# ORNL/DDStore

Hardware: AMD Instinct MI355X
Metric: samples/sec (global-shuffle sample fetch) (higher is better)
Workload: dtype bf16; 1 GPU; model=store-globalshuffle-fetch, global_batch=262144, rows_per_rank=2097152, row_bytes=512, store_dtype=f32, parallelism=dp1, mode=fetch

## Files before the change

ddstore_amd/csrc/ddstore_kernels.hip:

```cpp

#include "ddstore_kernels.h"

#include <hip/hip_fp16.h>
#include <hip/hip_bf16.h>
#include <hip/hip_fp8.h>
#include <type_traits>
#include <cstdlib>
#include <string>

namespace ddstore {

namespace {

constexpr int kBlock = 256;
constexpr int64_t kMaxBlocks = 32768;

inline int n_blocks(int64_t work_items) {
    int64_t b = (work_items + kBlock - 1) / kBlock;
    if (b < 1) b = 1;
    if (b > kMaxBlocks) b = kMaxBlocks;
    return (int)b;
}

template <typename T, int N>
struct alignas(sizeof(T) * N) VecT {
    T v[N];
};

__device__ __forceinline__ int owner_of(const int64_t* prefix, int nparts, int64_t row) {
    int lo = 0, hi = nparts - 1;
    while (lo < hi) {
        int mid = (lo + hi + 1) >> 1;
        if (prefix[mid] <= row) lo = mid; else hi = mid - 1;
    }
    return lo;
}

template <typename P, int NPFX = 1>
struct LdsDir {
    int64_t prefix[NPFX][DDS_MAX_PARTS + 1];
    P base[DDS_MAX_PARTS];

    __device__ __forceinline__ void load(const void* const* peer_base, int nparts,
                                         const int64_t* gprefix0,
                                         const int64_t* gprefix1 = nullptr) {
        for (int i = threadIdx.x; i <= nparts; i += kBlock) {
            prefix[0][i] = gprefix0[i];
            if constexpr (NPFX == 2) prefix[1][i] = gprefix1[i];
        }
        for (int i = threadIdx.x; i < nparts; i += kBlock)
            base[i] = reinterpret_cast<P>(peer_base[i]);
        __syncthreads();
    }
};

template <typename P, int NPFX>
__device__ __forceinline__ int owner_of(const LdsDir<P, NPFX>& d, int nparts, int64_t row) {
    return owner_of(d.prefix[0], nparts, row);
}

template <typename P, int NPFX>
__device__ __forceinline__ bool out_of_range(const LdsDir<P, NPFX>& d, int nparts,
                                             int64_t g) {
    return g < 0 || g >= d.prefix[0][nparts];
}

template <typename T>
constexpr bool is_fp8_v =
    std::is_same_v<T, __hip_fp8_e4m3> || std::is_same_v<T, __hip_fp8_e5m2>;

__device__ __forceinline__ float f64_to_f32(double v) {
#pragma clang fp contract(off)
    return static_cast<float>(v);
}

template <typename Tout, typename Tin>
__device__ __forceinline__ Tout cvt(Tin v) {
    if constexpr (std::is_same_v<Tout, Tin>) {
        return v;
    } else if constexpr (std::is_same_v<Tin, double> &&
                         (std::is_same_v<Tout, __half> ||
                          std::is_same_v<Tout, __hip_bfloat16>)) {
        return cvt<Tout, float>(f64_to_f32(v));
    } else if constexpr (std::is_same_v<Tout, uint8_t> &&
                         std::is_floating_point_v<Tin>) {
        return static_cast<uint8_t>(static_cast<int32_t>(v));
    } else if constexpr (std::is_same_v<Tin, __half>) {
        return cvt<Tout, float>(__half2float(v));
    } else if constexpr (std::is_same_v<Tin, __hip_bfloat16>) {
        return cvt<Tout, float>(__bfloat162float(v));
    } else if constexpr (is_fp8_v<Tin>) {
        return cvt<Tout, float>(static_cast<float>(v));
    } else if constexpr (std::is_same_v<Tout, __half>) {
        return __float2half(static_cast<float>(v));
    } else if constexpr (std::is_same_v<Tout, __hip_bfloat16>) {
        return __float2bfloat16(static_cast<float>(v));
    } else if constexpr (is_fp8_v<Tout>) {
        const float f = static_cast<float>(v);
        Tout r(f);
        if constexpr (std::is_same_v<Tout, __hip_fp8_e4m3>) {
            if (fabsf(f) > 464.0f) r.__x = 0x7F;
        } else {
            if (fabsf(f) >= 61440.0f) r.__x = f < 0.0f ? 0xFC : 0x7C;
        }
        return r;
    } else {
        return static_cast<Tout>(v);
    }
}

struct XfIdentity {
    template <typename Tout, typename Tin>
    __device__ __forceinline__ Tout apply(Tin v) const { return v; }
};
struct XfCast {
    template <typename Tout, typename Tin>
    __device__ __forceinline__ Tout apply(Tin v) const { return cvt<Tout>(v); }
};
struct XfAffine {
    float scale, shift;
    uint32_t opaque_zero = 0;
    template <typename Tout, typename Tin>
    __device__ __forceinline__ Tout apply(Tin v) const {
        float y = fmaf(cvt<float>(v), scale, shift);
        if constexpr (std::is_same_v<Tout, __half>)
            y = __uint_as_float(__float_as_uint(y) | opaque_zero);
        return cvt<Tout>(y);
    }
};

template <typename Tin, typename Tout, int VEC, typename Xf>
__global__ void __launch_bounds__(kBlock)
k_gather_oneshot(const void* const* peer_base, const int64_t* gprefix, int nparts,
                 const int64_t* idx, int64_t nidx, int64_t row_elems, Xf xf,
                 Tout* __restrict__ out, unsigned long long* oob) {
    using Vin = VecT<Tin, VEC>;
    using Vout = VecT<Tout, VEC>;
    __shared__ LdsDir<const Tin*> dir;
    dir.load(peer_base, nparts, gprefix);

    const int64_t cpr = row_elems / VEC;
    const int64_t total = nidx * cpr;
    for (int64_t t = (int64_t)blockIdx.x * kBlock + threadIdx.x; t < total;
         t += (int64_t)gridDim.x * kBlock) {
        const int64_t r = t / cpr;
        const int64_t c = t - r * cpr;
        const int64_t g = idx[r];
        if (out_of_range(dir, nparts, g)) {
            if (c == 0) atomicAdd(oob, 1ull);
            continue;
        }
        const int p = owner_of(dir, nparts, g);
        const Vin vin = *reinterpret_cast<const Vin*>(
            dir.base[p] + (g - dir.prefix[0][p]) * row_elems + c * VEC);
        Vout vout;
#pragma unroll
        for (int k = 0; k < VEC; ++k) vout.v[k] = xf.template apply<Tout>(vin.v[k]);
        *reinterpret_cast<Vout*>(out + t * VEC) = vout;
    }
}

typedef uint32_t dds_u32x4 __attribute__((ext_vector_type(4)));
typedef uint32_t dds_u32x2 __attribute__((ext_vector_type(2)));
#define DDS_GLOBAL_AS __attribute__((address_space(1)))

template <typename V>
__device__ __forceinline__ void store_out(V* p, const V& v) {
    static_assert(sizeof(V) == 16, "store side is exactly 16 B per lane");
    dds_u32x4 w;
    __builtin_memcpy(&w, &v, 16);
    __builtin_nontemporal_store(w, reinterpret_cast<dds_u32x4*>(p));
}

template <typename V>
__device__ __forceinline__ V load_global(uintptr_t a) {
    constexpr int B = sizeof(V);
    V r;
    if constexpr (B % 16 == 0) {
        dds_u32x4 w[B / 16];
#pragma unroll
        for (int i = 0; i < B / 16; ++i)
            w[i] = ((const DDS_GLOBAL_AS dds_u32x4*)a)[i];
        __builtin_memcpy(&r, w, B);
    } else if constexpr (B == 8) {
        const dds_u32x2 w = *(const DDS_GLOBAL_AS dds_u32x2*)a;
        __builtin_memcpy(&r, &w, B);
    } else if constexpr (B == 4) {
        const uint32_t w = *(const DDS_GLOBAL_AS uint32_t*)a;
        __builtin_memcpy(&r, &w, B);
    } else {
        static_assert(B == 2, "unsupported vector size");
        const uint16_t w = *(const DDS_GLOBAL_AS uint16_t*)a;
        __builtin_memcpy(&r, &w, B);
    }
    return r;
}

template <int INB>
constexpr int tiled_unroll() {
    return INB >= 128 ? 1 : (128 / INB > 8 ? 8 : 128 / INB);
}

template <typename Tin, typename Tout, typename Xf, bool LDSDIR>
__global__ void __launch_bounds__(kBlock)
k_gather_tiled(const GatherDirK dir, const void* const* peer_base,
               const int64_t* gprefix, int nparts,
               const int64_t* __restrict__ idx, int64_t nidx, int64_t ntiles,
               uint32_t cpr, uint32_t tile_rows, Xf xf,
               Tout* __restrict__ out, unsigned long long* oob) {
    constexpr int VEC = 16 / sizeof(Tout);
    constexpr int INB = VEC * sizeof(Tin);
    constexpr int U = tiled_unroll<INB>();
    using Vin = VecT<Tin, VEC>;
    using Vout = VecT<Tout, VEC>;
    __shared__ LdsDir<uintptr_t> ldir;
    if constexpr (LDSDIR) ldir.load(peer_base, nparts, gprefix);
    const int64_t total = LDSDIR ? ldir.prefix[0][nparts] : dir.prefix[DDS_DIR_KPARTS];

    const uint32_t lane = threadIdx.x & 63;
    const uint32_t wave = __builtin_amdgcn_readfirstlane(threadIdx.x >> 6);
    const int64_t wstride = (int64_t)gridDim.x * (kBlock / 64);
    int64_t tile = (int64_t)blockIdx.x * (kBlock / 64) + wave;
    if (tile >= ntiles) return;

    const uint32_t q64 = 64u / cpr, r64 = 64u % cpr;
    const uint32_t rl0 = lane / cpr, c0 = lane - rl0 * cpr;
    const int64_t row_bytes = (int64_t)cpr * INB;

    int64_t g_next = 0;
    {
        const int64_t r = tile * tile_rows + lane;
        if (lane < tile_rows && r < nidx) g_next = idx[r];
    }
    for (; tile < ntiles; tile += wstride) {
        const int64_t row0 = tile * tile_rows;
        const int64_t left = nidx - row0;
        const uint32_t nrows = left < (int64_t)tile_rows ? (uint32_t)left : tile_rows;
        const int64_t g = g_next;
        if (tile + wstride < ntiles) {
            const int64_t r = (tile + wstride) * tile_rows + lane;
            if (lane < tile_rows && r < nidx) g_next = idx[r];
        }
        uintptr_t src = 0;
        if (lane < nrows) {
            if (g < 0 || g >= total) {
                atomicAdd(oob, 1ull);
            } else if constexpr (LDSDIR) {
                const int p = owner_of(ldir, nparts, g);
                src = ldir.base[p] + (uintptr_t)((g - ldir.prefix[0][p]) * row_bytes);
            } else {
                int64_t pf = dir.prefix[0];
                uintptr_t bs = reinterpret_cast<uintptr_t>(dir.base[0]);
#pragma unroll
                for (int k = 1; k < DDS_DIR_KPARTS; ++k) {
                    const bool ge = dir.prefix[k] <= g;
                    pf = ge ? dir.prefix[k] : pf;
                    bs = ge ? reinterpret_cast<uintptr_t>(dir.base[k]) : bs;
                }
                src = bs + (uintptr_t)((g - pf) * row_bytes);
            }
        }
        Vout* __restrict__ op = reinterpret_cast<Vout*>(out) + row0 * cpr;
        const uint32_t nch = nrows * cpr;
        const bool clean = __ballot(lane < nrows && src == 0) == 0;
        uint32_t rl = rl0, c = c0;
        for (uint32_t jb = 0; jb < nch; jb += 64u * U) {
            if (clean && jb + 64u * U <= nch) {
                Vin vin[U];
#pragma unroll
                for (int u = 0; u < U; ++u) {
                    const uintptr_t sp =
                        (uintptr_t)__shfl((unsigned long long)src, (int)(rl & 63u));
                    vin[u] = load_global<Vin>(sp + (uintptr_t)(c * (uint32_t)INB));
                    c += r64;
                    rl += q64;
                    if (c >= cpr) {
                        c -= cpr;
                        rl += 1;
                    }
                }
#pragma unroll
                for (int u = 0; u < U; ++u) {
                    Vout vout;
#pragma unroll
                    for (int k = 0; k < VEC; ++k)
                        vout.v[k] = xf.template apply<Tout>(vin[u].v[k]);
                    store_out(&op[jb + 64u * u + lane], vout);
                }
            } else {
#pragma unroll 1
                for (int u = 0; u < U; ++u) {
                    const uint32_t j = jb + 64u * u + lane;
                    const uintptr_t sp =
                        (uintptr_t)__shfl((unsigned long long)src, (int)(rl & 63u));
                    if (j < nch && sp != 0) {
                        const Vin v =
                            load_global<Vin>(sp + (uintptr_t)(c * (uint32_t)INB));
                        Vout vout;
#pragma unroll
                        for (int k = 0; k < VEC; ++k)
                            vout.v[k] = xf.template apply<Tout>(v.v[k]);
                        store_out(&op[j], vout);
                    }
                    c += r64;
                    rl += q64;
                    if (c >= cpr) {
                        c -= cpr;
                        rl += 1;
                    }
                }
            }
        }
    }
}

__global__ void __launch_bounds__(kBlock)
k_csr_lens(const int64_t* goff, const int64_t* idx, int64_t nidx, int64_t nsamples,
           int64_t* __restrict__ lens, unsigned long long* oob,
           unsigned long long* elems) {
    int64_t acc = 0;
    for (int64_t i = (int64_t)blockIdx.x * kBlock + threadIdx.x; i < nidx;
         i += (int64_t)gridDim.x * kBlock) {
        const int64_t g = idx[i];
        if (g < 0 || g >= nsamples) {
            lens[i] = 0;
            atomicAdd(oob, 1ull);
            continue;
        }
        const int64_t L = goff[g + 1] - goff[g];
        lens[i] = L;
        acc += L;
    }
    if (elems) {
        for (int off = 32; off > 0; off >>= 1) acc += __shfl_down(acc, off);
        if ((threadIdx.x & 63) == 0 && acc)
            atomicAdd(elems, (unsigned long long)acc);
    }
}

__device__ __forceinline__ void copy_dwords_store16(
    uint32_t* __restrict__ dst, const uint32_t* __restrict__ src,
    int64_t nd, int tid, int nthreads) {
    const int64_t h_align = (int64_t)((4 - ((((uintptr_t)dst) >> 2) & 3)) & 3);
    const int64_t h = h_align < nd ? h_align : nd;
    for (int64_t i = tid; i < h; i += nthreads) dst[i] = src[i];
    const int64_t nb = (nd - h) >> 2;
    uint4* d4 = reinterpret_cast<uint4*>(dst + h);
    const uint32_t* s2 = src + h;
    for (int64_t i = tid; i < nb; i += nthreads) {
        uint4 o;
        o.x = s2[4 * i];
        o.y = s2[4 * i + 1];
        o.z = s2[4 * i + 2];
        o.w = s2[4 * i + 3];
        d4[i] = o;
    }
    for (int64_t i = h + (nb << 2) + tid; i < nd; i += nthreads) dst[i] = src[i];
}

template <typename U>
__device__ __forceinline__ void copy_units(U* dst, const U* src, int64_t n, int tid,
                                           int nthreads) {
    if constexpr (std::is_same_v<U, uint32_t>) {
        copy_dwords_store16(dst, src, n, tid, nthreads);
    } else {
        for (int64_t c = tid; c < n; c += nthreads) dst[c] = src[c];
    }
}

template <typename U, int GROUP>
__global__ void __launch_bounds__(kBlock)
k_gather_csr_wave(const void* const* peer_base,
                  const int64_t* sample_prefix, const int64_t* elem_prefix, int nparts,
                  const int64_t* goff,
                  const int64_t* idx, int64_t nidx,
                  const int64_t* out_off, int64_t units_per_elem,
                  int64_t cap_elems,
                  U* __restrict__ out, unsigned long long* ctrs) {
    __shared__ LdsDir<const U*, 2> dir;
    dir.load(peer_base, nparts, sample_prefix, elem_prefix);

    constexpr int GPB = kBlock / GROUP;
    const int64_t first = (int64_t)blockIdx.x * GPB + threadIdx.x / GROUP;
    const int64_t step = (int64_t)gridDim.x * GPB;
    const int tid = threadIdx.x % GROUP;
    for (int64_t s = first; s < nidx; s += step) {
        const int64_t g = idx[s];
        if (out_of_range(dir, nparts, g)) {
            if (tid == 0) atomicAdd(ctrs + DDS_CTR_OOB, 1ull);
            continue;
        }
        const int p = owner_of(dir, nparts, g);
        const int64_t e0 = goff[g];
        const int64_t len = goff[g + 1] - e0;
        const int64_t o0 = out_off[s];
        if (len <= 0) continue;
        if (o0 < 0 || o0 + len > cap_elems) {
            if (tid == 0) {
                atomicAdd(ctrs + DDS_CTR_CAP, 1ull);
                atomicAdd(ctrs + DDS_CTR_ELEMS,
                          (unsigned long long)(-(long long)len));
            }
            continue;
        }
        copy_units<U>(out + o0 * units_per_elem,
                      dir.base[p] + (e0 - dir.prefix[1][p]) * units_per_elem,
                      len * units_per_elem, tid, GROUP);
    }
}

constexpr int kItemBytes = 1024;

__device__ __forceinline__ void block_scan_pair(int64_t& x, int64_t& y,
                                                int64_t* s_wsum2, int lane,
                                                int wave, int64_t* tile_tot) {
    for (int off = 1; off < 64; off <<= 1) {
        int64_t ax = __shfl_up(x, off);
        int64_t ay = __shfl_up(y, off);
        if (lane >= off) {
            x += ax;
            y += ay;
        }
    }
    if (lane == 63) {
        s_wsum2[2 * wave] = x;
        s_wsum2[2 * wave + 1] = y;
    }
    __syncthreads();
    if (threadIdx.x == 0) {
        int64_t ax = 0, ay = 0;
        for (int w = 0; w < kBlock / 64; ++w) {
            int64_t tx = s_wsum2[2 * w], ty = s_wsum2[2 * w + 1];
            s_wsum2[2 * w] = ax;
            s_wsum2[2 * w + 1] = ay;
            ax += tx;
            ay += ty;
        }
        if (tile_tot) {
            tile_tot[0] = ax;
            tile_tot[1] = ay;
        }
    }
    __syncthreads();
    x += s_wsum2[2 * wave];
    y += s_wsum2[2 * wave + 1];
}

__global__ void __launch_bounds__(kBlock)
k_csr_plan1(const int64_t* goff, int64_t nsamples,
            const int64_t* idx, int64_t nidx, int64_t item_elems,
            int64_t* __restrict__ lens_tmp, int64_t* __restrict__ e0_tmp,
            int64_t* __restrict__ aggs, unsigned long long* ctrs) {
    __shared__ int64_t s_wsum2[2 * (kBlock / 64)];
    __shared__ int64_t s_tot[2];
    const int lane = threadIdx.x & 63;
    const int wave = threadIdx.x >> 6;
    const int64_t ntiles = (nidx + kBlock - 1) / kBlock;
    for (int64_t tile = blockIdx.x; tile < ntiles; tile += gridDim.x) {
        const int64_t i = tile * kBlock + threadIdx.x;
        int64_t L = 0, e0 = -1;
        if (i < nidx) {
            const int64_t g = idx[i];
            if (g < 0 || g >= nsamples) {
                atomicAdd(ctrs + DDS_CTR_OOB, 1ull);
            } else {
                e0 = goff[g];
                L = goff[g + 1] - e0;
            }
            lens_tmp[i] = L;
            e0_tmp[i] = e0;
        }
        int64_t x = L;
        int64_t y = L > 0 ? (L + item_elems - 1) / item_elems : 0;
        block_scan_pair(x, y, s_wsum2, lane, wave, s_tot);
        if (threadIdx.x == 0) {
            aggs[2 * tile] = s_tot[0];
            aggs[2 * tile + 1] = s_tot[1];
        }
        __syncthreads();
    }
}

__global__ void __launch_bounds__(kBlock)
k_csr_plan2(int64_t* __restrict__ aggs, int64_t ntiles,
            int64_t* __restrict__ meta, unsigned long long* ctrs) {
    __shared__ int64_t s_wsum2[2 * (kBlock / 64)];
    __shared__ int64_t s_tot[2];
    __shared__ int64_t s_carry[2];
    const int lane = threadIdx.x & 63;
    const int wave = threadIdx.x >> 6;
    if (threadIdx.x == 0) {
        s_carry[0] = 0;
        s_carry[1] = 0;
    }
    __syncthreads();
    for (int64_t base = 0; base < ntiles; base += kBlock) {
        const int64_t t = base + threadIdx.x;
        int64_t x = t < ntiles ? aggs[2 * t] : 0;
        int64_t y = t < ntiles ? aggs[2 * t + 1] : 0;
        const int64_t mx = x, my = y;
        block_scan_pair(x, y, s_wsum2, lane, wave, s_tot);
        if (t < ntiles) {
            aggs[2 * t] = s_carry[0] + x - mx;
            aggs[2 * t + 1] = s_carry[1] + y - my;
        }
        __syncthreads();
        if (threadIdx.x == 0) {
            s_carry[0] += s_tot[0];
            s_carry[1] += s_tot[1];
        }
        __syncthreads();
    }
    if (threadIdx.x == 0) {
        meta[0] = s_carry[1];
        meta[1] = s_carry[0];
        atomicAdd(ctrs + DDS_CTR_ELEMS, (unsigned long long)s_carry[0]);
    }
}

__global__ void __launch_bounds__(kBlock)
k_csr_plan3(const int64_t* __restrict__ lens_tmp,
            const int64_t* __restrict__ e0_tmp, int64_t nidx,
            const int64_t* sample_prefix, const int64_t* elem_prefix,
            int nparts, const int64_t* idx,
            int64_t item_elems, int64_t units_per_elem, int64_t cap_elems,
            const int64_t* __restrict__ aggs,
            int64_t* __restrict__ out_off,
            int64_t* __restrict__ desc, int64_t desc_cap,
            unsigned long long* ctrs) {
    __shared__ int64_t s_wsum2[2 * (kBlock / 64)];
    __shared__ int64_t s_sprefix[DDS_MAX_PARTS + 1];
    __shared__ int64_t s_eprefix[DDS_MAX_PARTS + 1];
    for (int i = threadIdx.x; i <= nparts; i += kBlock) {
        s_sprefix[i] = sample_prefix[i];
        s_eprefix[i] = elem_prefix[i];
    }
    __syncthreads();
    const int lane = threadIdx.x & 63;
    const int wave = threadIdx.x >> 6;
    const int64_t ntiles = (nidx + kBlock - 1) / kBlock;
    for (int64_t tile = blockIdx.x; tile < ntiles; tile += gridDim.x) {
        const int64_t i = tile * kBlock + threadIdx.x;
        const int64_t L = i < nidx ? lens_tmp[i] : 0;
        int64_t x = L;
        int64_t items = L > 0 ? (L + item_elems - 1) / item_elems : 0;
        int64_t y = items;
        block_scan_pair(x, y, s_wsum2, lane, wave, nullptr);
        const int64_t e_base = aggs[2 * tile], i_base = aggs[2 * tile + 1];
        if (i < nidx) {
            const int64_t excl_e = e_base + x - L;
            const int64_t excl_i = i_base + y - items;
            out_off[i + 1] = e_base + x;
            if (i == 0) out_off[0] = 0;
            if (L > 0) {
                if (excl_e + L > cap_elems ||
                    excl_i + items > desc_cap ||
                    L * units_per_elem >= (int64_t(1) << 44)) {
                    atomicAdd(ctrs + DDS_CTR_CAP, 1ull);
                    atomicAdd(ctrs + DDS_CTR_ELEMS,
                              (unsigned long long)(-(long long)L));
                    const int64_t end =
                        items < desc_cap - excl_i ? excl_i + items : desc_cap;
                    for (int64_t j = excl_i; j < end; ++j) {
                        desc[2 * j] = 0;
                        desc[2 * j + 1] = 0;
                    }
                } else {
                    const int64_t g = idx[i];
                    const int64_t p = owner_of(s_sprefix, nparts, g);
                    const int64_t src0 =
                        (e0_tmp[i] - s_eprefix[p]) * units_per_elem;
                    const int64_t dst0 = excl_e * units_per_elem;
                    const int64_t iu = item_elems * units_per_elem;
                    const int64_t nu = L * units_per_elem;
                    for (int64_t k = 0; k < items; ++k) {
                        const int64_t off = k * iu;
                        const int64_t n = nu - off < iu ? nu - off : iu;
                        desc[2 * (excl_i + k)] = (p << 56) | (src0 + off);
                        desc[2 * (excl_i + k) + 1] = (n << 44) | (dst0 + off);
                    }
                }
            }
        }
        __syncthreads();
    }
}

template <typename U, int GROUP>
__global__ void __launch_bounds__(kBlock)
k_gather_csr_items(const void* const* peer_base, int nparts,
                   const int64_t* __restrict__ desc,
                   const int64_t* __restrict__ meta, int64_t desc_cap,
                   U* __restrict__ out) {
    __shared__ const U* s_base[DDS_MAX_PARTS];
    for (int i = threadIdx.x; i < nparts; i += kBlock)
        s_base[i] = reinterpret_cast<const U*>(peer_base[i]);
    __syncthreads();
    const int64_t total = meta[0] < desc_cap ? meta[0] : desc_cap;
    constexpr int GPB = kBlock / GROUP;
    const int64_t first = (int64_t)blockIdx.x * GPB + threadIdx.x / GROUP;
    const int64_t step = (int64_t)gridDim.x * GPB;
    const int tid = threadIdx.x % GROUP;
    for (int64_t j = first; j < total; j += step) {
        const int64_t d0 = desc[2 * j];
        const int64_t d1 = desc[2 * j + 1];
        const int p = (int)(d0 >> 56);
        const int64_t src_u = d0 & ((int64_t(1) << 56) - 1);
        const int64_t n_u = d1 >> 44;
        const int64_t dst_u = d1 & ((int64_t(1) << 44) - 1);
        copy_units<U>(out + dst_u, s_base[p] + src_u, n_u, tid, GROUP);
    }
}

constexpr int kPadCountBlocks = 64;

template <typename P>
__device__ __forceinline__ void count_padded(const LdsDir<P, 2>& dir, int nparts,
                                             const int64_t* goff, const int64_t* idx,
                                             int64_t nidx, int64_t max_len,
                                             unsigned long long* s_acc,
                                             unsigned long long* ctrs) {
    const int64_t nb = gridDim.x < (unsigned)kPadCountBlocks ? gridDim.x : kPadCountBlocks;
    unsigned long long acc_elems = 0, acc_oob = 0;
    for (int64_t i = (int64_t)blockIdx.x * kBlock + threadIdx.x; i < nidx;
         i += nb * kBlock) {
        const int64_t g = idx[i];
        if (out_of_range(dir, nparts, g)) {
            acc_oob += 1;
        } else {
            const int64_t len = goff[g + 1] - goff[g];
            acc_elems += (unsigned long long)(len < max_len ? len : max_len);
        }
    }
    for (int off = 32; off > 0; off >>= 1) {
        acc_elems += __shfl_down(acc_elems, off);
        acc_oob += __shfl_down(acc_oob, off);
    }
    if ((threadIdx.x & 63) == 0) {
        s_acc[2 * (threadIdx.x >> 6)] = acc_elems;
        s_acc[2 * (threadIdx.x >> 6) + 1] = acc_oob;
    }
    __syncthreads();
    if (threadIdx.x == 0) {
        unsigned long long e = 0, o = 0;
        for (int w = 0; w < kBlock / 64; ++w) {
            e += s_acc[2 * w];
            o += s_acc[2 * w + 1];
        }
        if (e) atomicAdd(ctrs + DDS_CTR_ELEMS, e);
        if (o) atomicAdd(ctrs + DDS_CTR_OOB, o);
    }
}

template <typename Tin, typename Tout, int VEC, typename Xf>
__global__ void __launch_bounds__(kBlock)
k_gather_csr_padded(const void* const* peer_base, const int64_t* sample_prefix,
                    const int64_t* elem_prefix, int nparts, const int64_t* goff,
                    const int64_t* idx, int64_t nidx, int64_t disp, int64_t max_len,
                    int lg_group, bool aligned, Xf xf, dds_u32x4 pad16,
                    Tout* __restrict__ out, int64_t* __restrict__ lengths,
                    unsigned long long* ctrs) {
    using Vin = VecT<Tin, VEC>;
    using Vout = VecT<Tout, VEC>;
    static_assert(sizeof(Vout) <= 16, "pad16 covers one output chunk");
    __shared__ LdsDir<const Tin*, 2> dir;
    __shared__ unsigned long long s_acc[2 * (kBlock / 64)];
    dir.load(peer_base, nparts, sample_prefix, elem_prefix);

    Vout vpad;
    __builtin_memcpy(&vpad, &pad16, sizeof(Vout));
    const int group = 1 << lg_group;
    const int tid = threadIdx.x & (group - 1);
    const int64_t first =
        (int64_t)blockIdx.x * (kBlock >> lg_group) + (threadIdx.x >> lg_group);
    const int64_t step = (int64_t)gridDim.x * (kBlock >> lg_group);
    const int64_t row_elems = max_len * disp;
    const int64_t cpr = row_elems / VEC;
    if (blockIdx.x < kPadCountBlocks)
        count_padded(dir, nparts, goff, idx, nidx, max_len, s_acc, ctrs);
    for (int64_t s = first; s < nidx; s += step) {
        const int64_t g = idx[s];
        const Tin* sp = nullptr;
        int64_t nvalid = 0;
        if (out_of_range(dir, nparts, g)) {
            if (tid == 0) lengths[s] = 0;
        } else {
            const int p = owner_of(dir, nparts, g);
            const int64_t e0 = goff[g];
            const int64_t len = goff[g + 1] - e0;
            const int64_t take = len < max_len ? len : max_len;
            sp = dir.base[p] + (e0 - dir.prefix[1][p]) * disp;
            nvalid = take * disp;
            if (tid == 0) lengths[s] = len;
        }
        Vout* __restrict__ op = reinterpret_cast<Vout*>(out + s * row_elems);
        for (int64_t c = tid; c < cpr; c += group) {
            const int64_t e = c * VEC;
            Vout vout = vpad;
            if (e < nvalid) {
                if (VEC == 1 || aligned) {
                    const Vin vin = *reinterpret_cast<const Vin*>(sp + e);
#pragma unroll
                    for (int k = 0; k < VEC; ++k)
                        vout.v[k] = xf.template apply<Tout>(vin.v[k]);
                } else if (e + VEC <= nvalid) {
                    Tin x[VEC];
#pragma unroll
                    for (int k = 0; k < VEC; ++k) x[k] = sp[e + k];
#pragma unroll
                    for (int k = 0; k < VEC; ++k)
                        vout.v[k] = xf.template apply<Tout>(x[k]);
                } else {
#pragma unroll
                    for (int k = 0; k < VEC; ++k)
                        if (e + k < nvalid) vout.v[k] = xf.template apply<Tout>(sp[e + k]);
                }
            }
            op[c] = vout;
        }
    }
}


__global__ void __launch_bounds__(kBlock)
k_csr_scan3(const int64_t* __restrict__ lens_tmp, int64_t nidx,
            const int64_t* __restrict__ aggs, int64_t* __restrict__ out_off) {
    __shared__ int64_t s_wsum2[2 * (kBlock / 64)];
    const int lane = threadIdx.x & 63;
    const int wave = threadIdx.x >> 6;
    const int64_t ntiles = (nidx + kBlock - 1) / kBlock;
    for (int64_t tile = blockIdx.x; tile < ntiles; tile += gridDim.x) {
        const int64_t i = tile * kBlock + threadIdx.x;
        int64_t x = i < nidx ? lens_tmp[i] : 0;
        int64_t y = 0;
        block_scan_pair(x, y, s_wsum2, lane, wave, nullptr);
        if (i < nidx) {
            out_off[i + 1] = aggs[2 * tile] + x;
            if (i == 0) out_off[0] = 0;
        }
        __syncthreads();
    }
}

template <typename T>
struct IdPair {
    T src, dst;
};

constexpr int kGraphGroup = 64;

template <typename Tin, typename Tout, int GROUP, bool COO>
__global__ void __launch_bounds__(kBlock)
k_gather_csr_relabel(const void* const* peer_base, const int64_t* sample_prefix,
                     const int64_t* elem_prefix, int nparts, const int64_t* goff,
                     const int64_t* idx, int64_t nidx,
                     const int64_t* __restrict__ ptr,
                     const int64_t* __restrict__ edge_ptr, int64_t ncap,
                     int64_t ecap, Tout* __restrict__ out,
                     unsigned long long* ctrs) {
    using Pin = VecT<Tin, 2>;
    __shared__ LdsDir<const Pin*, 2> dir;
    dir.load(peer_base, nparts, sample_prefix, elem_prefix);

    constexpr int GPB = kBlock / GROUP;
    const int64_t first = (int64_t)blockIdx.x * GPB + threadIdx.x / GROUP;
    const int64_t step = (int64_t)gridDim.x * GPB;
    const int tid = threadIdx.x % GROUP;
    for (int64_t s = first; s < nidx; s += step) {
        const int64_t g = idx[s];
        if (out_of_range(dir, nparts, g)) continue;
        const int64_t o0 = edge_ptr[s];
        const int64_t len = edge_ptr[s + 1] - o0;
        if (len <= 0) continue;
        if (ptr[s + 1] > ncap || o0 < 0 || o0 + len > ecap) {
            if (tid == 0) {
                atomicAdd(ctrs + DDS_CTR_CAP, 1ull);
                atomicAdd(ctrs + DDS_CTR_ELEMS, (unsigned long long)(-(long long)len));
            }
            continue;
        }
        const Tout shift = static_cast<Tout>(ptr[s]);
        const int p = owner_of(dir, nparts, g);
        const Pin* __restrict__ sp = dir.base[p] + (goff[g] - dir.prefix[1][p]);
        for (int64_t e = tid; e < len; e += GROUP) {
            const Pin v = sp[e];
            const Tout a = static_cast<Tout>(v.v[0]) + shift;
            const Tout b = static_cast<Tout>(v.v[1]) + shift;
            if constexpr (COO) {
                out[o0 + e] = a;
                out[ecap + o0 + e] = b;
            } else {
                reinterpret_cast<IdPair<Tout>*>(out)[o0 + e] = IdPair<Tout>{a, b};
            }
        }
    }
}

template <typename T>
__device__ __forceinline__ void fill_store16(T* __restrict__ dst, int64_t n, T val,
                                             int64_t tid, int64_t nthreads) {
    constexpr int V = 16 / sizeof(T);
    using Vt = VecT<T, V>;
    const int64_t h_align =
        (int64_t)(((16 - ((uintptr_t)dst & 15)) & 15) / sizeof(T));
    const int64_t h = h_align < n ? h_align : n;
    for (int64_t i = tid; i < h; i += nthreads) dst[i] = val;
    const int64_t nb = (n - h) / V;
    Vt vv;
#pragma unroll
    for (int k = 0; k < V; ++k) vv.v[k] = val;
    Vt* d = reinterpret_cast<Vt*>(dst + h);
    for (int64_t i = tid; i < nb; i += nthreads) d[i] = vv;
    for (int64_t i = h + nb * V + tid; i < n; i += nthreads) dst[i] = val;
}

__device__ __forceinline__ int64_t block_last_le(const int64_t* __restrict__ a,
                                                 int64_t n, int64_t cap) {
    int64_t lo = 0, hi = n;
    while (hi > lo) {
        const int64_t m = hi - lo + 1;
        const int64_t stride = (m + kBlock - 1) / kBlock;
        const int64_t q = lo + (int64_t)threadIdx.x * stride;
        const int c = __syncthreads_count(q <= hi && a[q] <= cap);
        const int64_t nlo = lo + (int64_t)(c - 1) * stride;
        const int64_t nhi = nlo + stride - 1;
        lo = nlo;
        hi = nhi < hi ? nhi : hi;
    }
    return lo;
}

template <typename Tout, int GROUP>
__global__ void __launch_bounds__(kBlock)
k_graph_fill(const int64_t* __restrict__ ptr, const int64_t* __restrict__ edge_ptr,
             int64_t nidx, int64_t ncap, int64_t ecap, bool coo, Tout fill,
             int64_t* __restrict__ batch, Tout* __restrict__ edge_out) {
    const int64_t kn = block_last_le(ptr, nidx, ncap);
    const int64_t ke_all = block_last_le(edge_ptr, nidx, ecap);
    const int64_t ke = ke_all < kn ? ke_all : kn;
    const int64_t node_end = ptr[kn];
    const int64_t edge_end = edge_ptr[ke];

    constexpr int GPB = kBlock / GROUP;
    const int tid = threadIdx.x % GROUP;
    for (int64_t s = (int64_t)blockIdx.x * GPB + threadIdx.x / GROUP; s < kn;
         s += (int64_t)gridDim.x * GPB) {
        const int64_t o0 = ptr[s];
        fill_store16<int64_t>(batch + o0, ptr[s + 1] - o0, s, tid, GROUP);
    }
    const int64_t gt = (int64_t)blockIdx.x * kBlock + threadIdx.x;
    const int64_t nt = (int64_t)gridDim.x * kBlock;
    fill_store16<int64_t>(batch + node_end, ncap - node_end, nidx, gt, nt);
    if (coo) {
        fill_store16<Tout>(edge_out + edge_end, ecap - edge_end, fill, gt, nt);
        fill_store16<Tout>(edge_out + ecap + edge_end, ecap - edge_end, fill, gt, nt);
    } else {
        fill_store16<Tout>(edge_out + 2 * edge_end, 2 * (ecap - edge_end), fill, gt, nt);
    }
}

template <typename V>
__global__ void __launch_bounds__(kBlock)
k_scatter_rows(V* __restrict__ base, int64_t nrows, int64_t chunks_per_row,
               const int64_t* local_idx, int64_t nidx,
               const V* __restrict__ src, unsigned long long* oob) {
    const int64_t total = nidx * chunks_per_row;
    for (int64_t t = (int64_t)blockIdx.x * kBlock + threadIdx.x; t < total;
         t += (int64_t)gridDim.x * kBlock) {
        const int64_t r = t / chunks_per_row;
        const int64_t c = t - r * chunks_per_row;
        const int64_t l = local_idx[r];
        if (l < 0 || l >= nrows) {
            if (c == 0) atomicAdd(oob, 1ull);
            continue;
        }
        base[l * chunks_per_row + c] = src[t];
    }
}

inline int dds_itemsize(int t) {
    switch (t) {
        case DDS_U8: case DDS_F8E4M3: case DDS_F8E5M2: return 1;
        case DDS_F16: case DDS_BF16: return 2;
        case DDS_I32: case DDS_F32: return 4;
        default: return 8;
    }
}

struct DirArgs {
    const void* const* d_pb;
    const int64_t* d_pf;
    const void* const* h_pb;
    const int64_t* h_pf;
    int np;
};

struct GatherKnobs {
    int kernel = 0;
    int blocks = 0;
    bool dir_lds = false;
    int tile_rows = 64;
};
const GatherKnobs& gather_knobs() {
    static const GatherKnobs k = [] {
        GatherKnobs g;
        if (const char* e = getenv("DDSTORE_GATHER_KERNEL")) {
            const std::string s(e);
            g.kernel = s == "legacy" ? 1 : (s == "tiled" ? 2 : 0);
        }
        if (const char* e = getenv("DDSTORE_GATHER_BLOCKS")) {
            const int v = atoi(e);
            if (v > 0) g.blocks = v;
        }
        if (const char* e = getenv("DDSTORE_GATHER_DIR"))
            g.dir_lds = std::string(e) == "lds";
        if (const char* e = getenv("DDSTORE_GATHER_TILE_ROWS")) {
            const int v = atoi(e);
            if (v >= 1 && v <= 64) g.tile_rows = v;
        }
        return g;
    }();
    return k;
}

int cu_count() {
    static const int n = [] {
        int dev = 0, v = 0;
        if (hipGetDevice(&dev) != hipSuccess ||
            hipDeviceGetAttribute(&v, hipDeviceAttributeMultiprocessorCount, dev) !=
                hipSuccess || v <= 0)
            v = 256;
        return v;
    }();
    return n;
}

constexpr int kBlocksPerCU = 8;
constexpr int kTilesPerWave = 2;
constexpr int64_t kTiledMaxCpr = 4096;
constexpr int64_t kTiledMinCpr = 8;

template <typename Tin, typename Tout, typename Xf>
bool launch_tiled(hipStream_t stream, const DirArgs& d, const int64_t* idx,
                  int64_t n, int64_t re, Xf xf, Tout* out,
                  unsigned long long* oob) {
    constexpr int VEC = 16 / sizeof(Tout);
    constexpr int INB = VEC * (int)sizeof(Tin);
    constexpr int U = tiled_unroll<INB>();
    const GatherKnobs& kn = gather_knobs();
    if (kn.kernel == 1 || re % VEC != 0 || ((uintptr_t)out % 16) != 0) return false;
    const int64_t cpr = re / VEC;
    if (cpr > kTiledMaxCpr) return false;
    if (kn.kernel != 2 && cpr < kTiledMinCpr) return false;

    int64_t blocks_max = (int64_t)cu_count() * kBlocksPerCU;
    if (kn.blocks > 0) blocks_max = kn.blocks;
    int64_t tr_min = (64 * U + cpr - 1) / cpr;
    int64_t tr = n / (blocks_max * (kBlock / 64) * kTilesPerWave);
    if (tr < tr_min) tr = tr_min;
    if (tr > kn.tile_rows) tr = kn.tile_rows;
    const int64_t ntiles = (n + tr - 1) / tr;
    int64_t grid = (ntiles + (kBlock / 64) - 1) / (kBlock / 64);
    if (grid > blocks_max) grid = blocks_max;

    if (d.np <= DDS_DIR_KPARTS && !kn.dir_lds) {
        GatherDirK dir;
        const int64_t total = d.h_pf[d.np];
        for (int k = 0; k <= DDS_DIR_KPARTS; ++k)
            dir.prefix[k] = k < d.np ? d.h_pf[k] : total;
        for (int k = 0; k < DDS_DIR_KPARTS; ++k)
            dir.base[k] = k < d.np ? d.h_pb[k] : nullptr;
        hipLaunchKernelGGL((k_gather_tiled<Tin, Tout, Xf, false>), dim3((unsigned)grid),
                           dim3(kBlock), 0, stream, dir, d.d_pb, d.d_pf, d.np, idx, n,
                           ntiles, (uint32_t)cpr, (uint32_t)tr, xf, out, oob);
    } else {
        GatherDirK dir = {};
        hipLaunchKernelGGL((k_gather_tiled<Tin, Tout, Xf, true>), dim3((unsigned)grid),
                           dim3(kBlock), 0, stream, dir, d.d_pb, d.d_pf, d.np, idx, n,
                           ntiles, (uint32_t)cpr, (uint32_t)tr, xf, out, oob);
    }
    return true;
}

template <typename Tin, typename Tout, int VEC, typename Xf>
void launch_oneshot(hipStream_t stream, const DirArgs& d, const int64_t* idx,
                    int64_t n, int64_t re, Xf xf, Tout* out,
                    unsigned long long* oob) {
    const int grid = n_blocks(n * (re / VEC));
    hipLaunchKernelGGL((k_gather_oneshot<Tin, Tout, VEC, Xf>), dim3(grid), dim3(kBlock),
                       0, stream, d.d_pb, d.d_pf, d.np, idx, n, re, xf, out, oob);
}

template <typename Tin, typename Tout, typename Xf>
void launch_gather(hipStream_t stream, const DirArgs& d, const int64_t* idx,
                   int64_t n, int64_t re, Xf xf, Tout* out,
                   unsigned long long* oob) {
    constexpr int VEC = 16 / sizeof(Tout);
    if (launch_tiled<Tin, Tout>(stream, d, idx, n, re, xf, out, oob)) return;
    if (re % VEC == 0 && ((uintptr_t)out % 16) == 0)
        launch_oneshot<Tin, Tout, VEC>(stream, d, idx, n, re, xf, out, oob);
    else
        launch_oneshot<Tin, Tout, 1>(stream, d, idx, n, re, xf, out, oob);
}

template <typename T>
struct TypeTag {
    using type = T;
};

template <typename F>
void dispatch_dtype(int t, F&& f) {
    switch (t) {
        case DDS_U8: f(TypeTag<uint8_t>{}); break;
        case DDS_I32: f(TypeTag<int32_t>{}); break;
        case DDS_I64: f(TypeTag<int64_t>{}); break;
        case DDS_F32: f(TypeTag<float>{}); break;
        case DDS_F64: f(TypeTag<double>{}); break;
        case DDS_F16: f(TypeTag<__half>{}); break;
        case DDS_BF16: f(TypeTag<__hip_bfloat16>{}); break;
        case DDS_F8E4M3: f(TypeTag<__hip_fp8_e4m3>{}); break;
        case DDS_F8E5M2: f(TypeTag<__hip_fp8_e5m2>{}); break;
    }
}

template <int G0, int... Gs, typename F>
void dispatch_group(int group, F&& f) {
    if constexpr (sizeof...(Gs) == 0) {
        f(std::integral_constant<int, G0>{});
    } else {
        if (group == G0) f(std::integral_constant<int, G0>{});
        else dispatch_group<Gs...>(group, f);
    }
}

}

void gather_rows_affine(hipStream_t stream,
                        const void* const* d_peer_base,
                        const int64_t* d_prefix,
                        const void* const* h_peer_base,
                        const int64_t* h_prefix, int nparts,
                        const int64_t* d_idx, int64_t nidx,
                        int64_t row_elems, int in_t, int out_t,
                        float scale, float shift,
                        void* d_out, unsigned long long* d_oob) {
    if (nidx == 0 || row_elems == 0) return;
    const DirArgs dir{d_peer_base, d_prefix, h_peer_base, h_prefix, nparts};
    dispatch_dtype(in_t, [&](auto ti) {
        dispatch_dtype(out_t, [&](auto to) {
            using Tin = typename decltype(ti)::type;
            using Tout = typename decltype(to)::type;
            if constexpr (std::is_same_v<Tout, float> || std::is_same_v<Tout, __half> ||
                          std::is_same_v<Tout, __hip_bfloat16>)
                launch_gather<Tin, Tout>(stream, dir, d_idx, nidx, row_elems,
                                         XfAffine{scale, shift}, (Tout*)d_out, d_oob);
        });
    });
}

void gather_rows(hipStream_t stream,
                 const void* const* d_peer_base,
                 const int64_t* d_prefix,
                 const void* const* h_peer_base,
                 const int64_t* h_prefix, int nparts,
                 const int64_t* d_idx, int64_t nidx,
                 int64_t row_elems, int in_t, int out_t,
                 void* d_out, unsigned long long* d_oob) {
    if (nidx == 0 || row_elems == 0) return;
    const DirArgs dir{d_peer_base, d_prefix, h_peer_base, h_prefix, nparts};
    const int64_t row_bytes = row_elems * dds_itemsize(in_t);
    const uintptr_t out_align = (uintptr_t)d_out;
    if (in_t == out_t && row_bytes % 16 == 0 && out_align % 16 == 0) {
        if (launch_tiled<uint32_t, uint32_t>(stream, dir, d_idx, nidx, row_bytes / 4,
                                             XfIdentity{}, (uint32_t*)d_out, d_oob))
            return;
        using V32 = VecT<uint4, 2>;
        if (row_bytes % 32 == 0 && row_bytes >= 128 && out_align % 32 == 0)
            launch_oneshot<V32, V32, 1>(stream, dir, d_idx, nidx, row_bytes / 32,
                                        XfIdentity{}, (V32*)d_out, d_oob);
        else
            launch_oneshot<uint4, uint4, 1>(stream, dir, d_idx, nidx, row_bytes / 16,
                                            XfIdentity{}, (uint4*)d_out, d_oob);
        return;
    }
    dispatch_dtype(in_t, [&](auto ti) {
        dispatch_dtype(out_t, [&](auto to) {
            using Tin = typename decltype(ti)::type;
            using Tout = typename decltype(to)::type;
            launch_gather<Tin, Tout>(stream, dir, d_idx, nidx, row_elems, XfCast{},
                                     (Tout*)d_out, d_oob);
        });
    });
}

void csr_lens(hipStream_t stream, const int64_t* d_goff, const int64_t* d_idx,
              int64_t nidx, int64_t nsamples, int64_t* d_lens,
              unsigned long long* d_oob, unsigned long long* d_elems) {
    if (nidx == 0) return;
    hipLaunchKernelGGL(k_csr_lens, dim3(n_blocks(nidx)), dim3(kBlock), 0, stream,
                       d_goff, d_idx, nidx, nsamples, d_lens, d_oob, d_elems);
}


void gather_csr(hipStream_t stream,
                const void* const* d_peer_base,
                const int64_t* d_sample_prefix,
                const int64_t* d_elem_prefix, int nparts,
                const int64_t* d_goff,
                const int64_t* d_idx, int64_t nidx,
                const int64_t* d_out_off,
                int64_t elem_bytes, int64_t cap_elems,
                void* d_out, unsigned long long* d_ctrs) {
    if (nidx == 0) return;
    static const int g_override = [] {
        const char* e = getenv("DDSTORE_CSR_GROUP");
        return e ? atoi(e) : 0;
    }();
    int group = nidx >= 16384 ? 16 : (nidx >= 4096 ? 64 : 256);
    if (g_override) group = g_override;
    int64_t b = (nidx + (kBlock / group) - 1) / (kBlock / group);
    const int grid = (int)(b < kMaxBlocks ? b : kMaxBlocks);
    const uintptr_t oa = (uintptr_t)d_out;
    auto launch = [&](auto unit) {
        using U = typename decltype(unit)::type;
        dispatch_group<8, 16, 32, 64, 256>(group, [&](auto G) {
            hipLaunchKernelGGL((k_gather_csr_wave<U, G()>), dim3(grid), dim3(kBlock), 0,
                               stream, d_peer_base, d_sample_prefix, d_elem_prefix,
                               nparts, d_goff, d_idx, nidx, d_out_off,
                               elem_bytes / (int64_t)sizeof(U), cap_elems, (U*)d_out,
                               d_ctrs);
        });
    };
    if (elem_bytes % 16 == 0 && oa % 16 == 0) {
        launch(TypeTag<uint4>{});
    } else if (elem_bytes % 4 == 0 && oa % 4 == 0) {
        launch(TypeTag<uint32_t>{});
    } else {
        launch(TypeTag<uint8_t>{});
    }
}

void gather_csr_padded(hipStream_t stream, const void* const* d_peer_base,
                       const int64_t* d_sample_prefix,
                       const int64_t* d_elem_prefix, int nparts,
                       const int64_t* d_goff, int64_t nsamples_total,
                       const int64_t* d_idx, int64_t nidx,
                       int64_t row_elems, int64_t max_len, int in_t, int out_t,
                       bool affine, float scale, float shift, uint64_t pad_bits,
                       void* d_out, int64_t* d_lengths,
                       unsigned long long* d_ctrs) {
    if (nidx == 0) return;
    if (row_elems == 0 || max_len == 0) {
        hipLaunchKernelGGL(k_csr_lens, dim3(n_blocks(nidx)), dim3(kBlock), 0, stream,
                           d_goff, d_idx, nidx, nsamples_total, d_lengths,
                           d_ctrs + DDS_CTR_OOB, (unsigned long long*)nullptr);
        return;
    }
    const int osz = dds_itemsize(out_t);
    unsigned char pb[16];
    for (int i = 0; i < 16; ++i) pb[i] = (unsigned char)(pad_bits >> (8 * (i % osz)));
    dds_u32x4 pad16;
    __builtin_memcpy(&pad16, pb, 16);
    const uintptr_t oa = (uintptr_t)d_out;
    auto launch = [&](auto ti, auto to, auto vec, auto xf, int64_t disp, bool aligned) {
        using Tin = typename decltype(ti)::type;
        using Tout = typename decltype(to)::type;
        constexpr int VEC = decltype(vec)::value;
        const int64_t cpr = max_len * disp / VEC;
        int lg = cpr <= 8 ? 3 : (cpr <= 16 ? 4 : (cpr <= 32 ? 5 : 6));
        if (cpr > 64 && nidx < 4096) lg = 8;
        const int64_t gpb = kBlock >> lg;
        const int64_t b = (nidx + gpb - 1) / gpb;
        hipLaunchKernelGGL((k_gather_csr_padded<Tin, Tout, VEC, decltype(xf)>),
                           dim3((unsigned)(b < kMaxBlocks ? b : kMaxBlocks)),
                           dim3(kBlock), 0, stream, d_peer_base, d_sample_prefix,
                           d_elem_prefix, nparts, d_goff, d_idx, nidx, disp, max_len,
                           lg, aligned, xf, pad16, (Tout*)d_out, d_lengths, d_ctrs);
    };
    const int64_t elem_bytes = row_elems * dds_itemsize(in_t);
    if (!affine && in_t == out_t && elem_bytes % 16 == 0 && oa % 16 == 0) {
        launch(TypeTag<uint4>{}, TypeTag<uint4>{}, std::integral_constant<int, 1>{},
               XfIdentity{}, elem_bytes / 16, true);
        return;
    }
    auto launch_xf = [&](auto ti, auto to, auto xf) {
        using Tout = typename decltype(to)::type;
        constexpr int VEC = 16 / sizeof(Tout);
        if (oa % 16 == 0 && (max_len * row_elems) % VEC == 0)
            launch(ti, to, std::integral_constant<int, VEC>{}, xf, row_elems,
                   row_elems % VEC == 0);
        else
            launch(ti, to, std::integral_constant<int, 1>{}, xf, row_elems, true);
    };
    dispatch_dtype(in_t, [&](auto ti) {
        dispatch_dtype(out_t, [&](auto to) {
            using Tout = typename decltype(to)::type;
            if (!affine) {
                launch_xf(ti, to, XfCast{});
            } else if constexpr (std::is_same_v<Tout, float> ||
                                 std::is_same_v<Tout, __half> ||
                                 std::is_same_v<Tout, __hip_bfloat16>) {
                launch_xf(ti, to, XfAffine{scale, shift});
            }
        });
    });
}

size_t csr_plan_scratch_bytes(int64_t nidx) {
    const int64_t ntiles = (nidx + kBlock - 1) / kBlock;
    return (size_t)(2 * (ntiles > 0 ? ntiles : 1) + 2 * (nidx > 0 ? nidx : 1)
                    + 2) * sizeof(int64_t);
}

int64_t csr_item_elems(int64_t elem_bytes) {
    static const int item_bytes = [] {
        const char* e = getenv("DDSTORE_CSR_ITEM");
        int v = e ? atoi(e) : kItemBytes;
        return v >= 16 ? v : kItemBytes;
    }();
    int64_t ie = item_bytes / (elem_bytes > 0 ? elem_bytes : 1);
    return ie > 0 ? ie : 1;
}

void gather_csr_balanced(hipStream_t stream, const void* const* d_peer_base,
                         const int64_t* d_sample_prefix,
                         const int64_t* d_elem_prefix, int nparts,
                         const int64_t* d_goff, int64_t nsamples_total,
                         const int64_t* d_idx, int64_t nidx,
                         int64_t elem_bytes, int64_t cap_elems,
                         int64_t* d_out_off, void* d_out,
                         unsigned long long* d_ctrs,
                         void* d_scratch, int64_t* d_desc, int64_t desc_cap) {
    if (nidx == 0) return;
    const int64_t ntiles = (nidx + kBlock - 1) / kBlock;
    int64_t* aggs = reinterpret_cast<int64_t*>(d_scratch);
    int64_t* lens_tmp = aggs + 2 * ntiles;
    int64_t* e0_tmp = lens_tmp + nidx;
    int64_t* meta = e0_tmp + nidx;
    const int64_t item_elems = csr_item_elems(elem_bytes);
    const uintptr_t oa = (uintptr_t)d_out;
    const bool dw = elem_bytes % 4 == 0 && oa % 4 == 0;
    const int64_t upe = dw ? elem_bytes / 4 : elem_bytes;
    const int g1 = (int)(ntiles < kMaxBlocks ? ntiles : kMaxBlocks);
    hipLaunchKernelGGL(k_csr_plan1, dim3(g1), dim3(kBlock), 0, stream, d_goff,
                       nsamples_total, d_idx, nidx, item_elems, lens_tmp,
                       e0_tmp, aggs, d_ctrs);
    hipLaunchKernelGGL(k_csr_plan2, dim3(1), dim3(kBlock), 0, stream, aggs,
                       ntiles, meta, d_ctrs);
    hipLaunchKernelGGL(k_csr_plan3, dim3(g1), dim3(kBlock), 0, stream,
                       lens_tmp, e0_tmp, nidx, d_sample_prefix, d_elem_prefix,
                       nparts, d_idx, item_elems, upe, cap_elems, aggs,
                       d_out_off, d_desc, desc_cap, d_ctrs);
    static const int item_group = [] {
        const char* e = getenv("DDSTORE_CSR_ITEM_GROUP");
        int v = e ? atoi(e) : 16;
        return (v == 8 || v == 16 || v == 32) ? v : 16;
    }();
    const int64_t gi = (desc_cap + (kBlock / item_group) - 1)
                       / (kBlock / item_group);
    const int g2 = (int)(gi < kMaxBlocks ? gi : kMaxBlocks);
    auto launch = [&](auto unit, auto G) {
        using U = typename decltype(unit)::type;
        hipLaunchKernelGGL((k_gather_csr_items<U, G()>), dim3(g2), dim3(kBlock), 0,
                           stream, d_peer_base, nparts, d_desc, meta, desc_cap,
                           (U*)d_out);
    };
    if (dw) {
        dispatch_group<8, 32, 16>(item_group, [&](auto G) {
            launch(TypeTag<uint32_t>{}, G);
        });
    } else {
        launch(TypeTag<uint8_t>{}, std::integral_constant<int, 16>{});
    }
}

void csr_offsets(hipStream_t stream, const int64_t* d_goff, int64_t nsamples_total,
                 const int64_t* d_idx, int64_t nidx, int64_t* d_out_off,
                 void* d_scratch, unsigned long long* d_ctrs) {
    if (nidx == 0) return;
    const int64_t ntiles = (nidx + kBlock - 1) / kBlock;
    int64_t* aggs = reinterpret_cast<int64_t*>(d_scratch);
    int64_t* lens_tmp = aggs + 2 * ntiles;
    int64_t* e0_tmp = lens_tmp + nidx;
    int64_t* meta = e0_tmp + nidx;
    const int g1 = (int)(ntiles < kMaxBlocks ? ntiles : kMaxBlocks);
    hipLaunchKernelGGL(k_csr_plan1, dim3(g1), dim3(kBlock), 0, stream, d_goff,
                       nsamples_total, d_idx, nidx, (int64_t)1, lens_tmp, e0_tmp,
                       aggs, d_ctrs);
    hipLaunchKernelGGL(k_csr_plan2, dim3(1), dim3(kBlock), 0, stream, aggs,
                       ntiles, meta, d_ctrs);
    hipLaunchKernelGGL(k_csr_scan3, dim3(g1), dim3(kBlock), 0, stream, lens_tmp,
                       nidx, aggs, d_out_off);
}

void gather_csr_relabel(hipStream_t stream, const void* const* d_peer_base,
                        const int64_t* d_sample_prefix,
                        const int64_t* d_elem_prefix, int nparts,
                        const int64_t* d_goff, const int64_t* d_idx, int64_t nidx,
                        const int64_t* d_ptr, const int64_t* d_edge_ptr,
                        int64_t ncap, int64_t ecap, int in_t, int out_t, bool coo,
                        void* d_out, unsigned long long* d_ctrs) {
    if (nidx == 0) return;
    constexpr int G = kGraphGroup;
    const int64_t b = (nidx + (kBlock / G) - 1) / (kBlock / G);
    const int grid = (int)(b < kMaxBlocks ? b : kMaxBlocks);
    auto launch = [&](auto ti, auto to, auto c) {
        using Tin = typename decltype(ti)::type;
        using Tout = typename decltype(to)::type;
        hipLaunchKernelGGL((k_gather_csr_relabel<Tin, Tout, G, decltype(c)::value>),
                           dim3(grid), dim3(kBlock), 0, stream, d_peer_base,
                           d_sample_prefix, d_elem_prefix, nparts, d_goff, d_idx,
                           nidx, d_ptr, d_edge_ptr, ncap, ecap, (Tout*)d_out, d_ctrs);
    };
    auto launch_coo = [&](auto ti, auto to) {
        if (coo) launch(ti, to, std::true_type{});
        else launch(ti, to, std::false_type{});
    };
    if (in_t == DDS_I64 && out_t == DDS_I64)
        launch_coo(TypeTag<int64_t>{}, TypeTag<int64_t>{});
    else if (in_t == DDS_I32 && out_t == DDS_I64)
        launch_coo(TypeTag<int32_t>{}, TypeTag<int64_t>{});
    else if (in_t == DDS_I32 && out_t == DDS_I32)
        launch_coo(TypeTag<int32_t>{}, TypeTag<int32_t>{});
}

void graph_fill(hipStream_t stream, const int64_t* d_ptr, const int64_t* d_edge_ptr,
                int64_t nidx, int64_t ncap, int64_t ecap, int out_t, bool coo,
                int64_t edge_fill, int64_t* d_batch, void* d_edge_out) {
    if (ncap == 0 && ecap == 0) return;
    constexpr int G = kGraphGroup;
    const int64_t by_graph = (nidx + (kBlock / G) - 1) / (kBlock / G);
    const int64_t by_bytes =
        (ncap * 8 + 2 * ecap * (int64_t)dds_itemsize(out_t)) / (64 * kBlock) + 1;
    const int64_t b = by_graph > by_bytes ? by_graph : by_bytes;
    const int grid = (int)(b < kMaxBlocks ? b : kMaxBlocks);
    if (out_t == DDS_I64)
        hipLaunchKernelGGL((k_graph_fill<int64_t, G>), dim3(grid), dim3(kBlock), 0,
                           stream, d_ptr, d_edge_ptr, nidx, ncap, ecap, coo,
                           edge_fill, d_batch, (int64_t*)d_edge_out);
    else if (out_t == DDS_I32)
        hipLaunchKernelGGL((k_graph_fill<int32_t, G>), dim3(grid), dim3(kBlock), 0,
                           stream, d_ptr, d_edge_ptr, nidx, ncap, ecap, coo,
                           (int32_t)edge_fill, d_batch, (int32_t*)d_edge_out);
}

void scatter_rows_local(hipStream_t stream,
                        void* d_base, int64_t nrows_local,
                        int64_t row_elems, int elem_t,
                        const int64_t* d_local_idx, int64_t nidx,
                        const void* d_src, unsigned long long* d_oob) {
    if (nidx == 0 || row_elems == 0) return;
    const int64_t row_bytes = row_elems * dds_itemsize(elem_t);
    const uintptr_t al = (uintptr_t)d_src | (uintptr_t)d_base;
    auto launch = [&](auto chunk) {
        using V = typename decltype(chunk)::type;
        const int64_t cpr = row_bytes / (int64_t)sizeof(V);
        hipLaunchKernelGGL((k_scatter_rows<V>), dim3(n_blocks(nidx * cpr)),
                           dim3(kBlock), 0, stream, (V*)d_base, nrows_local, cpr,
                           d_local_idx, nidx, (const V*)d_src, d_oob);
    };
    if (row_bytes % 32 == 0 && row_bytes >= 128 && al % 32 == 0)
        launch(TypeTag<VecT<uint4, 2>>{});
    else if (row_bytes % 16 == 0 && al % 16 == 0)
        launch(TypeTag<uint4>{});
    else
        launch(TypeTag<uint8_t>{});
}

}
```

Before: 6.806 billion samples/s.

## Software-pipeline CSR item gather with prefetched descriptors and fixed vector chunks

Rewrites the dword path of the CSR item gather kernel. Each group now prefetches the next descriptor while the current item is copied, and short items are moved with a fixed set of four 16-byte vector loads plus one scalar tail, all issued before any store. Items too long for this fast path fall back to the generic copy. It also sets an occupancy hint in the launch bounds and adds an environment knob to cap the grid size. The aim is to hide descriptor and load latency, at the cost of more registers and a more complex mapping with clamped, predicated loads.

```diff
diff --git a/ddstore_amd/csrc/csr_item_map.h b/ddstore_amd/csrc/csr_item_map.h
--- /dev/null
+++ b/ddstore_amd/csrc/csr_item_map.h
@@ -0,0 +1,52 @@
+#pragma once
+
+#include <stdint.h>
+
+#if defined(__HIPCC__)
+#define DDS_MAP_FN __host__ __device__ inline
+#else
+#define DDS_MAP_FN inline
+#endif
+
+constexpr int kCsrItemCH = 4;
+
+struct CsrItemOp {
+    uint32_t load_off;
+    uint32_t store_off;
+    bool real;
+    bool store;
+};
+
+DDS_MAP_FN uint32_t csr_item_head(uint64_t dst_dw, int64_t n) {
+    const uint32_t a = (4u - (uint32_t)(dst_dw & 3u)) & 3u;
+    return (int64_t)a < n ? a : (uint32_t)n;
+}
+
+DDS_MAP_FN bool csr_item_fast(uint64_t dst_dw, int64_t n, int group) {
+    if (n <= 0) return true;
+    const int64_t nb = (n - csr_item_head(dst_dw, n)) >> 2;
+    return nb <= (int64_t)group * kCsrItemCH;
+}
+
+DDS_MAP_FN CsrItemOp csr_item_op(uint64_t dst_dw, uint32_t n, int group, int tid,
+                                 int k) {
+    const uint32_t h = csr_item_head(dst_dw, n);
+    const uint32_t nb = (n - h) >> 2;
+    CsrItemOp op;
+    if (k < kCsrItemCH) {
+        const uint32_t c = (uint32_t)(tid + k * group);
+        const uint32_t cc = c < nb ? c : nb - 1;
+        op.real = nb != 0;
+        op.store = c < nb;
+        op.load_off = op.real ? h + 4u * cc : 0u;
+        op.store_off = h + 4u * c;
+    } else {
+        const uint32_t t = n - h - 4u * nb;
+        const uint32_t e = (uint32_t)tid;
+        const uint32_t o = e < h ? e : 4u * nb + e;
+        op.real = op.store = e < h + t;
+        op.load_off = op.real ? o : 0u;
+        op.store_off = o;
+    }
+    return op;
+}
diff --git a/ddstore_amd/csrc/ddstore_kernels.hip b/ddstore_amd/csrc/ddstore_kernels.hip
--- a/ddstore_amd/csrc/ddstore_kernels.hip
+++ b/ddstore_amd/csrc/ddstore_kernels.hip
@@ -1,5 +1,6 @@
 
 #include "ddstore_kernels.h"
+#include "csr_item_map.h"
 
 #include <hip/hip_fp16.h>
 #include <hip/hip_bf16.h>
@@ -586,8 +587,10 @@
     }
 }
 
+typedef uint32_t dds_u32x4_a4 __attribute__((ext_vector_type(4), aligned(4)));
+
 template <typename U, int GROUP>
-__global__ void __launch_bounds__(kBlock)
+__global__ void __launch_bounds__(kBlock, 6)
 k_gather_csr_items(const void* const* peer_base, int nparts,
                    const int64_t* __restrict__ desc,
                    const int64_t* __restrict__ meta, int64_t desc_cap,
@@ -598,17 +601,68 @@
     __syncthreads();
     const int64_t total = meta[0] < desc_cap ? meta[0] : desc_cap;
     constexpr int GPB = kBlock / GROUP;
-    const int64_t first = (int64_t)blockIdx.x * GPB + threadIdx.x / GROUP;
     const int64_t step = (int64_t)gridDim.x * GPB;
     const int tid = threadIdx.x % GROUP;
-    for (int64_t j = first; j < total; j += step) {
-        const int64_t d0 = desc[2 * j];
-        const int64_t d1 = desc[2 * j + 1];
-        const int p = (int)(d0 >> 56);
-        const int64_t src_u = d0 & ((int64_t(1) << 56) - 1);
-        const int64_t n_u = d1 >> 44;
-        const int64_t dst_u = d1 & ((int64_t(1) << 44) - 1);
-        copy_units<U>(out + dst_u, s_base[p] + src_u, n_u, tid, GROUP);
+    constexpr int64_t kLow56 = (int64_t(1) << 56) - 1, kLow44 = (int64_t(1) << 44) - 1;
+    if constexpr (!std::is_same_v<U, uint32_t>) {
+        const int64_t first = (int64_t)blockIdx.x * GPB + threadIdx.x / GROUP;
+        for (int64_t j = first; j < total; j += step) {
+            const int64_t d0 = desc[2 * j];
+            const int64_t d1 = desc[2 * j + 1];
+            const int p = (int)(d0 >> 56);
+            copy_units<U>(out + (d1 & kLow44), s_base[p] + (d0 & kLow56), d1 >> 44, tid,
+                          GROUP);
+        }
+    } else {
+        constexpr int CH = kCsrItemCH;
+        const int wave = __builtin_amdgcn_readfirstlane(threadIdx.x >> 6);
+        int64_t jw = (int64_t)blockIdx.x * GPB + wave * (64 / GROUP);
+        if (jw >= total) return;
+        const int64_t last = total - 1;
+        int64_t j = jw + (threadIdx.x & 63) / GROUP;
+        int64_t jj = j < last ? j : last;
+        int64_t d0 = desc[2 * jj], d1 = desc[2 * jj + 1];
+        asm volatile("" : "+v"(d0), "+v"(d1));
+        for (; jw < total; jw += step, j += step) {
+            const int p = (int)(d0 >> 56);
+            const int64_t src_u = d0 & kLow56;
+            const int64_t n_u = j < total ? d1 >> 44 : 0;
+            const int64_t dst_u = d1 & kLow44;
+            const uintptr_t slot = (uintptr_t)(desc + 2 * jj);
+            if (jw + step < total) {
+                jj = j + step < last ? j + step : last;
+                d0 = desc[2 * jj];
+                d1 = desc[2 * jj + 1];
+            }
+            uint32_t* dp = out + dst_u;
+            const uint64_t dst_dw = (uint64_t)((uintptr_t)dp >> 2);
+            if (__ballot(!csr_item_fast(dst_dw, n_u, GROUP)) != 0) {
+                copy_units<U>(dp, s_base[p] + src_u, n_u, tid, GROUP);
+                continue;
+            }
+            const uintptr_t sa = (uintptr_t)(s_base[p] + src_u);
+            CsrItemOp op[CH + 1];
+            dds_u32x4 v[CH];
+#pragma unroll
+            for (int k = 0; k <= CH; ++k)
+                op[k] = csr_item_op(dst_dw, (uint32_t)n_u, GROUP, tid, k);
+#pragma unroll
+            for (int k = 0; k < CH; ++k)
+                v[k] = *(const DDS_GLOBAL_AS dds_u32x4_a4*)(
+                    op[k].real ? sa + 4 * (uintptr_t)op[k].load_off : slot);
+            uint32_t e = load_global<uint32_t>(
+                op[CH].real ? sa + 4 * (uintptr_t)op[CH].load_off : slot);
+            asm volatile(""
+                         : "+v"(v[0]), "+v"(v[1]), "+v"(v[2]), "+v"(v[3]), "+v"(e),
+                           "+v"(d0), "+v"(d1)
+                         :
+                         : "memory");
+            static_assert(CH == 4, "the wait above names every chunk");
+#pragma unroll
+            for (int k = 0; k < CH; ++k)
+                if (op[k].store) *reinterpret_cast<dds_u32x4*>(dp + op[k].store_off) = v[k];
+            if (op[CH].store) dp[op[CH].store_off] = e;
+        }
     }
 }
 
@@ -1256,8 +1310,13 @@
         int v = e ? atoi(e) : 16;
         return (v == 8 || v == 16 || v == 32) ? v : 16;
     }();
-    const int64_t gi = (desc_cap + (kBlock / item_group) - 1)
-                       / (kBlock / item_group);
+    static const int item_blocks = [] {
+        const char* e = getenv("DDSTORE_CSR_ITEM_BLOCKS");
+        const int v = e ? atoi(e) : 0;
+        return v > 0 ? v : 0;
+    }();
+    int64_t gi = (desc_cap + (kBlock / item_group) - 1) / (kBlock / item_group);
+    if (item_blocks > 0 && gi > item_blocks) gi = item_blocks;
     const int g2 = (int)(gi < kMaxBlocks ? gi : kMaxBlocks);
     auto launch = [&](auto unit, auto G) {
         using U = typename decltype(unit)::type;
```

Result: no change. 6.804 billion samples/s (-0.0%).
